# jixinya/EAMM

Hardware: AMD Instinct MI355X
Metric: 256x256 frames/sec (dense-motion + generator forward) (higher is better)
Workload: dtype f32; 1 GPU; 256x256, 10 keypoints, batch=16 synthetic frames per GPU per step, source encoded once per clip (BASELINE.json configs[2]); parallelism=frame-sharded x1

## Files before the change

eamm_amd/csrc/api_common.h:

```cpp
#pragma once
#include "../../include/eamm_hip.h"
#include "kernels.h"

#include <algorithm>
#include <cmath>
#include <cstdarg>
#include <cstdio>
#include <cstdlib>
#include <cstring>
#include <map>
#include <string>
#include <vector>

namespace eamm {

inline thread_local std::string g_create_error;

namespace {

struct HostTensor {
    std::vector<int64_t> shape;
    std::vector<float> data;
    size_t numel() const {
        size_t n = 1;
// ... 13 lines not shown


struct CtxBase {
    int device = 0;
    std::string err;
    std::map<std::string, HostTensor> sd;
    bool finalized = false;
    std::vector<void*> owned;
    int dma_min_m = 4608;
    int big_min_m = 49152;
    int dma_cfg_n256 = 2, dma_cfg_n128 = 2, dma_cfg_n64 = 3;
    int patch_poly = 1;
    int skinny_max_m = 16384;
    int patch_split_max = 4;
    int patch_min_blocks = 128;
};

struct DeviceGuard {
    int prev = -1;
    bool switched = false;
    hipError_t status = hipSuccess;
    explicit DeviceGuard(int device) {
        if (hipGetDevice(&prev) != hipSuccess) prev = -1;
        if (prev != device) {
            status = hipSetDevice(device);
            switched = status == hipSuccess && prev >= 0;
        }
    }
    ~DeviceGuard() {
        if (switched) (void)hipSetDevice(prev);
// ... 285 lines not shown
    if (int rc = fold_conv(c, {{conv, norm}}, 3, Cin_real, &f)) return rc;
    HostConv p = f;
    p.Cin = Cin_packed;
    p.w.assign((size_t)f.Cout * Cin_packed * 9, 0.f);
    for (int o = 0; o < f.Cout; ++o)
        std::copy_n(f.w.begin() + (size_t)o * Cin_real * 9, (size_t)Cin_real * 9, p.w.begin() + (size_t)o * Cin_packed * 9);
    return pack_wino(c, p, 4, L, false);
}

const ConvLayer& pick(const CtxBase* c, const LayerSet& S, size_t M) {
    if (S.has_skinny && M <= (size_t)c->skinny_max_m) return M <= 32 ? S.skinny32 : S.skinny64;
    if (S.has_big && M >= (size_t)c->big_min_m) return S.big;
    return (S.has_dma && M >= (size_t)c->dma_min_m) ? S.dma : S.base;
}

int launch_up(CtxBase* c, const LayerSet& S, const ConvIO& io, hipStream_t s) {
    if (S.has_patch) {
        int cus = 256;
        (void)hipDeviceGetAttribute(&cus, hipDeviceAttributeMultiprocessorCount, c->device);
        int splits = 1;
        if (S.patch.w_poly) {
            splits = patch_poly_splits(S.patch, io.B, io.Hin, io.Win, c->patch_split_max, cus);
            if ((size_t)splits * io.B * 4 * io.Hin * io.Win * S.patch.Cout > io.partial_cap) splits = 1;
        }
        const int blocks = ((io.Hin + 15) / 16) * ((io.Win + 15) / 16) * io.B * ((S.patch.Cout + 31) / 32) * splits;
        if (blocks >= c->patch_min_blocks && io.Hin >= 16 && io.Win >= 16 && io.act == ACT_RELU && !io.resid && !io.out2 && !io.pool && !io.nchw) {
            if (S.patch.w_poly)
                HIP_TRY(c, patch_poly_launch(S.patch, io.in0, io.in1, io.B, io.Hin, io.Win, io.act, io.out, s, splits, io.partial,
                                             io.partial_cap));
            else
                HIP_TRY(c, patch_phase_launch(S.patch, io.in0, io.in1, io.B, io.Hin, io.Win, io.act, io.out, s));
            return EAMM_OK;
        }
    }
    HIP_TRY(c, conv_launch(pick(c, S, (size_t)io.B * io.Hin * io.Win), io, s));
    return EAMM_OK;
}

int env_int(const char* name, int dflt) { return (int)knob_int(name, dflt); }

int round_up(int v, int m) { return (v + m - 1) / m * m; }

bool is_pow2(int v) { return v > 0 && (v & (v - 1)) == 0; }


inline void read_tile_knobs(CtxBase* c) {
    c->dma_min_m = env_int("EAMM_DMA_MIN_M", c->dma_min_m);
    c->big_min_m = env_int("EAMM_BIG_MIN_M", c->big_min_m);
    c->patch_poly = env_int("EAMM_PATCH_POLY", c->patch_poly);
    c->dma_cfg_n256 = env_int("EAMM_DMA_CFG_N256", c->dma_cfg_n256);
    c->dma_cfg_n128 = env_int("EAMM_DMA_CFG_N128", c->dma_cfg_n128);
    c->dma_cfg_n64 = env_int("EAMM_DMA_CFG_N64", c->dma_cfg_n64);
    c->patch_min_blocks = env_int("EAMM_PATCH_MIN_BLOCKS", c->patch_min_blocks);
    c->patch_split_max = env_int("EAMM_PATCH_SPLIT_MAX", c->patch_split_max);
    c->skinny_max_m = env_int("EAMM_SKINNY_MAX_M", c->skinny_max_m);
}

inline void free_owned(CtxBase* c) {
    DeviceGuard guard(c->device);
    (void)hipDeviceSynchronize();
    for (void* p : c->owned) (void)hipFree(p);
    c->owned.clear();
}

inline int store_tensor(CtxBase* c, const char* key, const float* host, const int64_t* shape, int ndim) {
    if (!c || !key || !host || ndim < 0 || (ndim > 0 && !shape)) return fail(c, EAMM_ERR_ARG, "null argument");
    if (c->finalized) return fail(c, EAMM_ERR_STATE, "weights already finalised; create a new handle to reload");
    HostTensor t;
    t.shape.assign(shape, shape + ndim);
// ... 29 lines not shown
```

eamm_amd/csrc/conv_mfma_patch_poly.hip:

```cpp
#include "conv_common.h"

#include <algorithm>
#include <cstdlib>
#include <cstring>

namespace eamm {

typedef __attribute__((address_space(3))) void* lds_ptr_t;

__device__ __forceinline__ f32x4 pk_sub4(f32x4 a, f32x4 b) {
    typedef float f32x2 __attribute__((ext_vector_type(2)));
    f32x2 alo = {a[0], a[1]}, ahi = {a[2], a[3]}, blo = {b[0], b[1]}, bhi = {b[2], b[3]}, rlo, rhi;
    asm("v_pk_add_f32 %0, %1, %2 neg_lo:[0,1] neg_hi:[0,1]" : "=v"(rlo) : "v"(alo), "v"(blo));
    asm("v_pk_add_f32 %0, %1, %2 neg_lo:[0,1] neg_hi:[0,1]" : "=v"(rhi) : "v"(ahi), "v"(bhi));
    return f32x4{rlo[0], rlo[1], rhi[0], rhi[1]};
}

namespace {
constexpr int ZT = 16;
constexpr int ZW = ZT + 2;
constexpr int ZPIX = ZW * ZW;
constexpr int ZPAD = (ZPIX + 7) / 8 * 8;
constexpr int ZBN = 32;
constexpr int ZWAVES = 8;
// ... 1 lines not shown

struct PatchPolyArgs {
    const float* in0;
    const float* in1;
    int C0, C1;
    unsigned in0_bytes, in1_bytes, w_bytes;
    int B, H, W;
    int tiles_x, tiles_y, ntiles;
    const float* w;
    const float* bias;
    int Cout, act;
    float* out;
    int splits;
    float* partial;
    size_t slab;
};

template <int FORM>
__global__ __launch_bounds__(ZWAVES * 64) void conv_patch_poly_kernel(const PatchPolyArgs p) {
    constexpr int BK = CONV_BK;
    constexpr int A_STAGE = ZPAD * BK;
    constexpr int B_STAGE = 9 * ZBN * BK;
    constexpr int A_PIECES = ZPAD / 8, B_PIECES = 9 * ZBN / 8;
    constexpr int A_INSTR = (A_PIECES + ZWAVES - 1) / ZWAVES;
    constexpr int B_INSTR = (B_PIECES + ZWAVES - 1) / ZWAVES;
    static_assert(A_INSTR + B_INSTR <= 12, "one DMA piece per sub-step");
    constexpr int B3_STAGE = 9 * 3 * 256;
    constexpr int B3_PIECES = 9 * 3, B3_INSTR = (B3_PIECES + ZWAVES - 1) / ZWAVES, A_HALF = A_INSTR / 2;
    static_assert(A_INSTR % 2 == 0 && B3_INSTR + A_HALF <= 9, "one DMA piece per point of a half-chunk");
    extern __shared__ __attribute__((aligned(16))) float smem[];
    float* const As = smem;
    float* const Bs = smem + 2 * A_STAGE;

    const int tid = threadIdx.x;
    const int lane = tid & 63;
    const int wave = __builtin_amdgcn_readfirstlane(tid >> 6);
    const int l31 = lane & 31, half = lane >> 5;

    int L = xcd_remap(blockIdx.x, gridDim.x);
    const int ntile = L % p.ntiles;
    L /= p.ntiles;
    const int ks = L % p.splits;
    L /= p.splits;
    const int tx0 = (L % p.tiles_x) * ZT;
    L /= p.tiles_x;
    const int ty0 = (L % p.tiles_y) * ZT;
    const int b = L / p.tiles_y;
    const int cchunks = (p.C0 + p.C1) / BK;
    const int c_begin = ks * cchunks / p.splits, c_end = (ks + 1) * cchunks / p.splits;

    const __amdgpu_buffer_rsrc_t rs0 = __builtin_amdgcn_make_buffer_rsrc((void*)p.in0, 0, p.in0_bytes, 0x00020000);
    const __amdgpu_buffer_rsrc_t rs1 =
        __builtin_amdgcn_make_buffer_rsrc((void*)(p.in1 ? p.in1 : p.in0), 0, p.in1 ? p.in1_bytes : 0u, 0x00020000);
    const __amdgpu_buffer_rsrc_t rsw = __builtin_amdgcn_make_buffer_rsrc((void*)p.w, 0, p.w_bytes, 0x00020000);
    constexpr unsigned OOB = 0xFFFFFFF0u;
    int pix[A_INSTR];
    static_for<A_INSTR>([&](auto jc) {
        constexpr int j = decltype(jc)::value;
        const int i = (wave + ZWAVES * j) * 8 + (lane >> 3);
        const int pyy = i / ZW, pxx = i - pyy * ZW;
        const int y = ty0 + pyy - 1, x = tx0 + pxx - 1;
        const bool ok = i < ZPIX && (unsigned)y < (unsigned)p.H && (unsigned)x < (unsigned)p.W;
        pix[j] = ok ? (b * p.H + y) * p.W + x : -1;
    });
    const unsigned slot_b = (unsigned)(((lane & 7) ^ ((((wave & 1) << 2) + (lane >> 4)) & 7)) << 4);
    auto dma_patch_piece = [&](auto jc, int cc, int st) {
        constexpr int j = decltype(jc)::value;
        if (wave + ZWAVES * j < A_PIECES) {
            const int c0 = cc * BK;
            const bool first = c0 < p.C0;
            const int C = first ? p.C0 : p.C1;
            const unsigned so = (unsigned)(first ? c0 : c0 - p.C0) * 4u;
            const int pj = pix[j];
            const unsigned vo = pj >= 0 ? (unsigned)(pj * C) * 4u + slot_b : OOB;
            float* dst = As + st * A_STAGE + (wave + ZWAVES * j) * (8 * BK);
            __builtin_amdgcn_raw_ptr_buffer_load_lds(first ? rs0 : rs1, (lds_ptr_t)dst, 16, vo, so, 0, 0);
        }
    };
    const unsigned w_lane = (unsigned)lane * 16u;
    auto dma_weight_piece = [&](auto jc, int cc, int st) {
        constexpr int j = decltype(jc)::value;
        if (wave + ZWAVES * j < B_PIECES) {
            const unsigned so = (unsigned)((ntile * cchunks + cc) * B_STAGE + (wave + ZWAVES * j) * (8 * BK)) * 4u;
            float* dst = Bs + st * B_STAGE + (wave + ZWAVES * j) * (8 * BK);
            __builtin_amdgcn_raw_ptr_buffer_load_lds(rsw, (lds_ptr_t)dst, 16, w_lane, so, 0, 0);
        }
    };

    auto dma_plane_piece = [&](auto jc, int hc, int wst) {
        constexpr int j = decltype(jc)::value;
        if (wave + ZWAVES * j < B3_PIECES) {
            const unsigned so = (unsigned)((ntile * 2 * cchunks + hc) * B3_STAGE + (wave + ZWAVES * j) * 256) * 4u;
            float* dst = Bs + wst * B3_STAGE + (wave + ZWAVES * j) * 256;
            __builtin_amdgcn_raw_ptr_buffer_load_lds(rsw, (lds_ptr_t)dst, 16, w_lane, so, 0, 0);
        }
    };

    f32x16 acc[9];
    static_for<9>([&](auto kc) {
        static_for<16>([&](auto rc) { acc[decltype(kc)::value][decltype(rc)::value] = 0.f; });
    });

    const int trow = 2 * wave + (l31 >> 4), tcol = ((l31 & 15) - 2 * (l31 >> 4)) & 15;
    const int idx0 = (trow + 1) * ZW + tcol + 1;
    int ta[9];
    static_for<9>([&](auto kc) {
        constexpr int k = decltype(kc)::value;
        const int idx = idx0 + (k / 3 - 1) * ZW + (k % 3 - 1);
        ta[k] = idx * BK + ((half ^ ((idx >> 1) & 7)) << 2);
    });
    const int bw0 = l31 * BK + ((half ^ ((l31 >> 1) & 7)) << 2);

    f32x4 x1[3];
    f32x4 xr[3];
    f32x4 v[2][3];
    f32x4 bb[2][3];
// ... 18 lines not shown
        v[q & 1][0] = r1;
        v[q & 1][1] = r0 - r1;
        v[q & 1][2] = r2 - r1;
    };
    auto mfmas = [&](auto qc, auto hc) {
        constexpr int q = decltype(qc)::value, i = q % 3, h = decltype(hc)::value;
        static_for<2>([&](auto tc) {
            constexpr int t = 2 * h + decltype(tc)::value;
            static_for<3>([&](auto jc) {
                constexpr int j = decltype(jc)::value;
                acc[3 * i + j] = __builtin_amdgcn_mfma_f32_32x32x2f32(v[q & 1][j][t], bb[q & 1][j][t], acc[3 * i + j], 0, 0, 0);
            });
        });
    };

    auto chunk = [&](int cc) {
        const int st = (cc - c_begin) & 1;
        const float* a_stage = As + st * A_STAGE;
        const float* b_stage = Bs + st * B_STAGE;
        const bool more = cc + 1 < c_end;
        fetch(std::integral_constant<int, 0>{}, a_stage, b_stage);
        transform(std::integral_constant<int, 0>{});
        static_for<12>([&](auto qc) {
            constexpr int q = decltype(qc)::value;
            if constexpr (q + 1 < 12) fetch(std::integral_constant<int, q + 1>{}, a_stage, b_stage);
            __builtin_amdgcn_sched_barrier(0);
            mfmas(qc, std::integral_constant<int, 0>{});
            __builtin_amdgcn_sched_barrier(0);
            if constexpr (q + 1 < 12) transform(std::integral_constant<int, q + 1>{});
            __builtin_amdgcn_sched_barrier(0);
            mfmas(qc, std::integral_constant<int, 1>{});
            if constexpr (q < B_INSTR) {
                if (more) dma_weight_piece(std::integral_constant<int, q>{}, cc + 1, st ^ 1);
            } else if constexpr (q - B_INSTR < A_INSTR) {
                if (more) dma_patch_piece(std::integral_constant<int, q - B_INSTR>{}, cc + 1, st ^ 1);
            }
            __builtin_amdgcn_sched_barrier(0);
        });
        asm volatile("s_waitcnt vmcnt(0)" ::: "memory");
        __syncthreads();
    };

    auto half_chunk = [&](int cc, auto Sc) {
        constexpr int S = decltype(Sc)::value;
        const int st = (cc - c_begin) & 1;
        const float* a_stage = As + st * A_STAGE;
        const float* b_stage = Bs + S * B3_STAGE + lane * 4;
        const bool more = cc + 1 < c_end;
        f32x4 xr[2], cr[2], r1[2];
        u32x4 ap[3], ub[3];
        auto load_raw = [&](auto ptc) {
            constexpr int pt = decltype(ptc)::value, i = pt / 3, j = pt % 3;
            constexpr int col = j == 0 ? 1 : j == 1 ? 0 : 2, row = i == 0 ? 1 : i == 1 ? 0 : 2;
            static_for<2>([&](auto hc) {
                constexpr int h2 = decltype(hc)::value;
                xr[h2] = *reinterpret_cast<const f32x4*>(a_stage + (ta[3 * row + col] ^ (8 * (2 * S + h2))));
                if constexpr (i > 0) cr[h2] = *reinterpret_cast<const f32x4*>(a_stage + (ta[3 + col] ^ (8 * (2 * S + h2))));
            });
        };
        auto load_planes = [&](auto ptc) {
            constexpr int pt = decltype(ptc)::value;
            static_for<3>([&](auto plc) {
                constexpr int pl = decltype(plc)::value;
// ... 14 lines not shown
        static_for<9>([&](auto ptc) {
            constexpr int pt = decltype(ptc)::value;
            load_planes(ptc);
            __builtin_amdgcn_sched_barrier(0);
            split_point(ptc);
            __builtin_amdgcn_sched_barrier(0);
            if constexpr (pt + 1 < 9) load_raw(std::integral_constant<int, pt + 1>{});
            __builtin_amdgcn_sched_barrier(0);
            static_for<SPLIT_TERMS>([&](auto tc) {
                constexpr int t = decltype(tc)::value;
                constexpr int pa = SPLIT_TERM_A[t], pb = SPLIT_TERM_B[t];
                acc[pt] = __builtin_amdgcn_mfma_f32_32x32x16_bf16(__builtin_bit_cast(bf16x8_t, ap[pa]),
                                                                  __builtin_bit_cast(bf16x8_t, ub[pb]), acc[pt], 0, 0, 0);
            });
            if constexpr (pt < B3_INSTR) {
                if (S == 0 || more) dma_plane_piece(std::integral_constant<int, pt>{}, 2 * cc + S + 1, S ^ 1);
            } else if constexpr (pt - B3_INSTR < A_HALF) {
                if (more) dma_patch_piece(std::integral_constant<int, A_HALF * S + pt - B3_INSTR>{}, cc + 1, st ^ 1);
            }
            __builtin_amdgcn_sched_barrier(0);
        });
        asm volatile("s_waitcnt vmcnt(0)" ::: "memory");
        __syncthreads();
    };

    static_for<A_INSTR>([&](auto jc) { dma_patch_piece(jc, c_begin, 0); });
    if constexpr (FORM == 1) static_for<B3_INSTR>([&](auto jc) { dma_plane_piece(jc, 2 * c_begin, 0); });
    else static_for<B_INSTR>([&](auto jc) { dma_weight_piece(jc, c_begin, 0); });
    asm volatile("s_waitcnt vmcnt(0)" ::: "memory");
    __syncthreads();
    if constexpr (FORM == 1) {
        for (int cc = c_begin; cc < c_end; ++cc) {
            half_chunk(cc, std::integral_constant<int, 0>{});
            half_chunk(cc, std::integral_constant<int, 1>{});
        }
    } else {
        for (int cc = c_begin; cc < c_end; ++cc) chunk(cc);
    }

    constexpr int LDO = ZBN + 4, C4 = ZBN / 4, NTHR = ZWAVES * 64, PER = ZT * ZT * C4 / NTHR;
    const int OH = 2 * p.H, OW = 2 * p.W;
    const bool raw = p.splits > 1;
    const float bias = raw ? 0.f : p.bias[ntile * ZBN + l31];
    float* const dst = raw ? p.partial + (size_t)ks * p.slab : p.out;
    static_for<4>([&](auto phc) {
        constexpr int ph = decltype(phc)::value, py = ph >> 1, px = ph & 1;
        if constexpr (ph > 0) __syncthreads();
        static_for<16>([&](auto rc) {
            constexpr int r = decltype(rc)::value;
            const int m = (r & 3) + 8 * (r >> 2) + 4 * half;
            const int pixel = (2 * wave + (m >> 4)) * ZT + (((m & 15) - 2 * (m >> 4)) & 15);
            const float y = (acc[0][r] + acc[1 + px][r]) + (acc[3 * (1 + py)][r] + acc[3 * (1 + py) + 1 + px][r]);
            smem[pixel * LDO + l31] = y + bias;
        });
        __syncthreads();
#pragma unroll
        for (int k = 0; k < PER; ++k) {
            const int idx = tid + k * NTHR;
            const int row = idx / C4, c4 = idx - row * C4;
            const int y = ty0 + (row >> 4), x = tx0 + (row & 15);
            const int n = ntile * ZBN + c4 * 4;
            if (y < p.H && x < p.W && n < p.Cout) {
                float4 o4 = *reinterpret_cast<const float4*>(smem + row * LDO + c4 * 4);
                if (!raw) {
                    o4.x = apply_act(o4.x, p.act); o4.y = apply_act(o4.y, p.act);
                    o4.z = apply_act(o4.z, p.act); o4.w = apply_act(o4.w, p.act);
                }
                const size_t o = ((size_t)(b * OH + 2 * y + py) * OW + 2 * x + px) * p.Cout + n;
                *reinterpret_cast<float4*>(dst + o) = o4;
            }
        }
    });
}

__global__ __launch_bounds__(256) void patch_poly_reduce_kernel(const float* __restrict__ partial, int splits, size_t slab,
                                                                const float* __restrict__ bias, int Cout, int act,
                                                                float* __restrict__ out, size_t total4) {
    const int c4n = Cout >> 2;
    for (size_t i = (size_t)blockIdx.x * blockDim.x + threadIdx.x; i < total4; i += (size_t)gridDim.x * blockDim.x) {
        float4 v = reinterpret_cast<const float4*>(partial)[i];
        for (int sp = 1; sp < splits; ++sp) {
            const float4 t = reinterpret_cast<const float4*>(partial + (size_t)sp * slab)[i];
            v.x += t.x; v.y += t.y; v.z += t.z; v.w += t.w;
        }
        const float4 bs = reinterpret_cast<const float4*>(bias)[i % c4n];
        v.x = apply_act(v.x + bs.x, act); v.y = apply_act(v.y + bs.y, act);
        v.z = apply_act(v.z + bs.z, act); v.w = apply_act(v.w + bs.w, act);
// ... 54 lines not shown
    const size_t total = 3 * patch_poly_packed_elems(cin_packed, Cout);
    for (size_t i = 0; i < total; ++i) dst[i] = 0;
    patch_poly_for_each_u(w, Cout, Cin, cin_map, cin_packed, [&](int o, int cp, int pt, float u) {
        const int nt = o / ZBN, nl = o % ZBN;
        const int hc = cp / 16, kl = cp % 16;
        const int lane = ((kl >> 2) & 1) * 32 + nl, e = (kl >> 3) * 4 + (kl & 3);
        uint16_t pl[3];
        split3_bf16_host(u, pl);
        uint16_t* blk = dst + ((((size_t)nt * hch + hc) * 9 + pt) * 3) * 512 + lane * 8 + e;
        for (int k = 0; k < 3; ++k) blk[k * 512] = pl[k];
    });
}

size_t patch_poly_split_packed_elems(int Cin_packed, int Cout) { return patch_poly_packed_elems(Cin_packed, Cout) * 3 / 2; }

hipError_t patch_poly_launch(const PatchLayer& L, const float* in0, const float* in1, int B, int H, int W, int act,
                              float* out, hipStream_t stream, int splits, float* partial, size_t partial_cap) {
    if ((L.C0 % CONV_BK) || (L.C1 % CONV_BK) || (L.Cout & 3) || L.w_poly == nullptr) return hipErrorInvalidValue;
    const size_t slab = (size_t)B * 4 * H * W * L.Cout;
    if (splits < 1 || (splits > 1 && (partial == nullptr || (size_t)splits * slab > partial_cap))) return hipErrorInvalidValue;
    PatchPolyArgs a{};
    a.in0 = in0;
    a.in1 = L.C1 ? in1 : nullptr;
    a.C0 = L.C0;
    a.C1 = L.C1;
    const size_t px = (size_t)B * H * W;
    const bool split = splits == 1 && L.w_poly3 != nullptr;
    const size_t b0 = px * L.C0 * 4, b1 = px * L.C1 * 4,
                 bw = (split ? patch_poly_split_packed_elems(L.C0 + L.C1, L.Cout) : patch_poly_packed_elems(L.C0 + L.C1, L.Cout)) * 4;
    if (b0 >= 0xFFFFFFF0ull || b1 >= 0xFFFFFFF0ull || bw >= 0xFFFFFFF0ull) return hipErrorInvalidValue;
    a.in0_bytes = (unsigned)b0;
    a.in1_bytes = (unsigned)b1;
    a.w_bytes = (unsigned)bw;
    a.B = B;
    a.H = H;
    a.W = W;
    a.tiles_x = (W + ZT - 1) / ZT;
    a.tiles_y = (H + ZT - 1) / ZT;
    a.ntiles = (L.Cout + ZBN - 1) / ZBN;
    a.w = split ? L.w_poly3 : L.w_poly;
    a.bias = L.bias;
    a.Cout = L.Cout;
    a.act = act;
    a.out = out;
    a.splits = splits;
    a.partial = partial;
    a.slab = slab;
    constexpr size_t lds_loop0 = sizeof(float) * 2 * (ZPAD * CONV_BK + 9 * ZBN * CONV_BK);
    constexpr size_t lds_loop1 = sizeof(float) * 2 * (ZPAD * CONV_BK + 9 * 3 * 256);
    constexpr size_t lds_epi = sizeof(float) * (ZT * ZT) * (ZBN + 4);
    static_assert(lds_loop0 <= 160 * 1024 && lds_loop0 >= lds_loop1 && lds_loop1 >= lds_epi, "LDS budget");
    const size_t lds = split ? lds_loop1 : lds_loop0;
    static lds_once_mask configured[2] = {{0}, {0}};
    const auto kern = split ? conv_patch_poly_kernel<1> : conv_patch_poly_kernel<0>;
    if (hipError_t e = ensure_dynamic_lds(kern, lds, &configured[split]); e != hipSuccess) return e;
    const int blocks = a.tiles_x * a.tiles_y * B * a.ntiles * splits;
    note_mfma_flops(2.0 * a.tiles_x * a.tiles_y * B * (ZT * ZT) * 9.0 * (a.ntiles * ZBN) * (L.C0 + L.C1));
    hipLaunchKernelGGL(kern, dim3(blocks), dim3(ZWAVES * 64), lds, stream, a);
    if (splits > 1) {
        const size_t total4 = slab / 4;
        const int rb = (int)std::min<size_t>((total4 + 255) / 256, 4096);
        hipLaunchKernelGGL(patch_poly_reduce_kernel, dim3(rb), dim3(256), 0, stream, partial, splits, slab, L.bias, L.Cout, act, out,
                           total4);
    }
    return hipGetLastError();
}

}
```

eamm_amd/csrc/eamm_forward.hip:

```cpp
#include "eamm_ctx.h"
#include <mutex>

namespace {
constexpr int POOL_MAXDEV = 64, POOL_MAXCHAIN = 15;
std::mutex g_pool_mu;
hipStream_t g_pool[POOL_MAXDEV][POOL_MAXCHAIN] = {};
std::mutex g_pool_lease[POOL_MAXDEV];

}

hipStream_t chain_stream(int device, int k) {
    if (device < 0 || device >= POOL_MAXDEV || k < 0 || k >= POOL_MAXCHAIN) return nullptr;
    std::lock_guard<std::mutex> lock(g_pool_mu);
    if (!g_pool[device][k] && hipStreamCreateWithFlags(&g_pool[device][k], hipStreamNonBlocking) != hipSuccess) g_pool[device][k] = nullptr;
    return g_pool[device][k];
}

FrameView make_view(const eamm_ctx* c, int f0, int n, int ns_call, int slab, const float* kd_val, const float* kd_jac,
                    const float* ks_val, const float* ks_jac, const eamm_outputs* o) {
    FrameView v;
    const size_t F = (size_t)f0, K = c->K;
    const size_t HW = (size_t)c->H * c->W, hw = (size_t)c->h * c->w, hwf = (size_t)c->hf * c->wf;
    const size_t sf = ns_call > 1 ? F : 0;
    v.n = n;
// ... 412 lines not shown
    const eamm_outputs* const user = o;
    eamm_outputs staged = *o;
    if (o->frames_u8 && c->Cimg != 3) return fail(c, EAMM_ERR_ARG, "uint8 RGB frames need num_channels == 3");
    if (c->Cimg < 3) {
        if (o->frames_u8) return fail(c, EAMM_ERR_ARG, "uint8 RGB frames need num_channels == 3");
        staged.prediction = c->stage_pred;
        if (o->deformed) staged.deformed = c->stage_deformed;
        if (o->sparse_deformed) staged.sparse_deformed = c->stage_sparse;
        o = &staged;
    }

    StreamLease lease(c, s);
    if (lease.rc) return lease.rc;
    const int chains = pass_chains(c, n);
    c->cur_call_frames = n;
    c->prof.begin_call(n, chains);
    if (chains == 1) {
        if (int rc = forward_view(c, make_view(c, 0, n, ns, 0, kd_val, kd_jac, ks_val, ks_jac, o), s, 0, false)) return rc;
    } else {
        const int nbase = n / chains, nrem = n % chains;
        HIP_TRY(c, hipEventRecord(c->ev_fork, s));
        for (int k = 1; k < chains; ++k) HIP_TRY(c, hipStreamWaitEvent(c->side_streams[k - 1], c->ev_fork, 0));
        for (int k = 0; k < chains; ++k) {
            const int nk = nbase + (k < nrem ? 1 : 0), f0 = k * nbase + std::min(k, nrem);
            const FrameView v = make_view(c, f0, nk, ns, k, kd_val, kd_jac, ks_val, ks_jac, o);
            if (int rc = forward_view(c, v, k ? c->side_streams[k - 1] : s, k, true)) return rc;
        }
        for (int k = 1; k < chains; ++k) {
            HIP_TRY(c, hipEventRecord(c->ev_join[k - 1], c->side_streams[k - 1]));
            HIP_TRY(c, hipStreamWaitEvent(s, c->ev_join[k - 1], 0));
// ... 146 lines not shown
```

eamm_amd/csrc/eamm_op_conv.hip:

```cpp
#include "op_common.h"

namespace {

struct ConvOp {
    const float *in0, *in1;
    int C0, C1, B, Hin, Win, up;
    const float *w, *b;
    int Cout, kh, kw, act, pool;
    const float* resid;
    int splitk, tile_n;
    float* out;
    int iters;
    float* avg_ms;
    const float *pre_s, *pre_t;
    float* out2;
    const float *s2, *t2;
    int nchw, split_n;
    const char* name;
    hipStream_t s;
};

const char* conv_refusal(const ConvOp& a) {
    const bool staged = a.tile_n == 0 || a.tile_n == 32 || a.tile_n == 64 || a.tile_n == 128;
    const bool gemm = staged || (a.tile_n > 1000 && a.tile_n <= 1005);
// ... 52 lines not shown
    if (a.kh != 7 || a.kw != 1 || a.up || a.pool || a.resid || a.splitk > 1 || a.Cout != bn || a.act != 0 || a.C0 % 32 || a.C1 % 32 ||
        (!streamed && (a.C1 || a.C0 > 64)))
        return fail(t, EAMM_ERR_ARG, "%s: unsupported column-patch configuration", a.name);
    float* w = nullptr;
    if (int rc = upload_conv_image(t, &w, op_weights(a, a.C0 + a.C1, false), nullptr, a.C0 + a.C1, bn, MODE_PLAIN, true)) return rc;
    auto col7 = [&]() {
        return streamed ? conv_col7s_launch(a.in0, a.C0, a.in1, a.C1, a.B, a.Hin, a.Win, w, 3, a.out, 96, a.s)
                        : conv_col7_launch(a.in0, a.C0, a.B, a.Hin, a.Win, w, a.out, a.s);
    };
    HIP_TRY(t, col7());
    HIP_TRY(t, time_launches(a.s, a.iters, a.avg_ms, col7));
    return EAMM_OK;
}

int op_conv_patch(OpBuffers* t, const ConvOp& a) {
    const bool pp = a.tile_n == 3003 || a.tile_n == 3004;
    const int psplit = a.splitk > 1 ? a.splitk : 1;
    if (a.kh != 3 || a.kw != 3 || !a.up || a.pool || a.resid || (a.Cout & 3) || (psplit > 1 && (!pp || ((a.C0 + a.C1) / 32) % psplit)))
        return fail(t, EAMM_ERR_ARG, "%s: unsupported patch-kernel configuration", a.name);
    PatchLayer P;
    float* ppart = nullptr;
    const size_t ppart_elems = psplit > 1 ? (size_t)psplit * a.B * 4 * a.Hin * a.Win * a.Cout : 0;
    int rc = pack_patch(t, op_weights(a, a.C0 + a.C1), nullptr, a.C0, a.C1, pp, &P, a.tile_n == 3003);
    if (rc || (psplit > 1 && (rc = dev_alloc(t, &ppart, ppart_elems)))) return rc;
    auto patch = [&]() {
        return pp ? patch_poly_launch(P, a.in0, a.in1, a.B, a.Hin, a.Win, a.act, a.out, a.s, psplit, ppart, ppart_elems)
                  : patch_phase_launch(P, a.in0, a.in1, a.B, a.Hin, a.Win, a.act, a.out, a.s);
    };
    HIP_TRY(t, patch());
    HIP_TRY(t, time_launches(a.s, a.iters, a.avg_ms, patch));
    return EAMM_OK;
}

int op_conv_wino(OpBuffers* t, const ConvOp& a) {
    const bool w4 = a.tile_n >= 2100;
    const int w4_groups = a.tile_n >= 2150 ? a.tile_n - 2150 : 1;
    const int w4_variant = w4_groups > 1 ? 0 : a.tile_n - 2100;
    if ((!w4 && a.tile_n != 2000) || a.kh != 3 || a.kw != 3 || a.up || (a.pool && (w4_groups == 1 || a.resid)) || a.C1 || a.splitk > 1 || a.C0 % 64 ||
        (a.Cout & 3) || (w4 && ((a.Hin & 3) || (a.Win & 3))))
        return fail(t, EAMM_ERR_ARG, "%s: unsupported Winograd configuration", a.name);
    WinoLayer W;
    float *V = nullptr, *Zb = nullptr;
    int rc = pack_wino(t, op_weights(a, a.C0), w4 ? 4 : 2, &W);
    if (rc || (rc = dev_alloc(t, &V, (size_t)16 * a.B * (a.Hin / 2) * (a.Win / 2) * a.C0))) return rc;
// ... 37 lines not shown
    io.out2 = a.out2;
    io.s2 = a.s2;
    io.t2 = a.t2;
    io.split_n = a.split_n;
    if (io.partial_cap && (rc = dev_alloc(t, &io.partial, io.partial_cap))) return rc;
    auto gemm = [&]() { return conv_launch(L, io, a.s, a.splitk); };
    HIP_TRY(t, gemm());
    HIP_TRY(t, time_launches(a.s, a.iters, a.avg_ms, gemm));
    return EAMM_OK;
}

int op_conv_run(OpBuffers* t, const ConvOp& a) {
    int rc;
    if (a.tile_n == 4002 || a.tile_n == 4003) rc = op_conv_final(t, a);
    else if (a.tile_n == 4000 || a.tile_n == 4001) rc = op_conv_col7(t, a);
    else if (a.tile_n == 3000 || a.tile_n == 3003 || a.tile_n == 3004) rc = op_conv_patch(t, a);
    else if (a.tile_n >= 2000 && a.tile_n < 2200) rc = op_conv_wino(t, a);
    else rc = op_conv_gemm(t, a);
    if (rc) return rc;
    HIP_TRY(t, hipStreamSynchronize(a.s));
    return EAMM_OK;
}

int op_conv_call(int device, ConvOp a, void* stream_) {
    if (const char* why = conv_refusal(a)) return fail(nullptr, EAMM_ERR_ARG, "%s: %s", a.name, why);
    DeviceGuard guard(device);
    if (guard.status != hipSuccess) return fail(nullptr, EAMM_ERR_HIP, "hipSetDevice failed");
    a.s = reinterpret_cast<hipStream_t>(stream_);
    OpBuffers t(device, a.s);
    if (int rc = op_conv_run(&t, a)) return fail(nullptr, rc, "%s", t.err.c_str());
    return EAMM_OK;
// ... 84 lines not shown
```

eamm_amd/csrc/kernels.h:

```cpp
#pragma once
#include <hip/hip_runtime.h>
#include <stddef.h>
#include <stdint.h>

namespace eamm {

constexpr int CONV_BK = 32;
constexpr int CONV_LDK = CONV_BK + 4;
inline size_t round64(size_t n) { return (n + 63) / 64 * 64; }
constexpr int KP_STRIDE = 8;

enum Act { ACT_NONE = 0, ACT_RELU = 1, ACT_SIGMOID = 2 };

void note_mfma_flops(double flops);
double take_mfma_flops();
double total_mfma_flops();

long long knob_int(const char* name, long long dflt);
int knobs_json(char* buf, int cap);

struct ConvArgs {
    const float* in0;
    const float* in1;
    int C0, C1;
// ... 59 lines not shown
hipError_t conv_launch(const ConvLayer& L, const ConvIO& io, hipStream_t stream, int force_splits = 0);

struct PatchLayer {
    int C0 = 0, C1 = 0, Cout = 0;
    float* w = nullptr;
    float* w_poly = nullptr;
    float* w_poly3 = nullptr;
    float* bias = nullptr;
};
size_t patch_packed_elems(int Cin_packed, int Cout);
size_t patch_poly_packed_elems(int Cin_packed, int Cout);
void patch_poly_pack_host(const float* w_oihw_3x3, int Cout, int Cin, const int* cin_map, int cin_packed, float* dst);
size_t patch_poly_split_packed_elems(int Cin_packed, int Cout);
void patch_poly_pack_split_host(const float* w_oihw_3x3, int Cout, int Cin, const int* cin_map, int cin_packed, uint16_t* dst);
hipError_t patch_poly_launch(const PatchLayer& L, const float* in0, const float* in1, int B, int H, int W, int act,
                             float* out, hipStream_t stream, int splits = 1, float* partial = nullptr, size_t partial_cap = 0);
int patch_poly_splits(const PatchLayer& L, int B, int H, int W, int max_splits, int cus);
void patch_pack_host(const float* w_oihw_3x3, int Cout, int Cin, const int* cin_map, int cin_packed, float* dst);
hipError_t patch_phase_launch(const PatchLayer& L, const float* in0, const float* in1, int B, int H, int W, int act,
                              float* out, hipStream_t stream);

hipError_t conv_col7_launch(const float* in, int C, int B, int H, int W, const float* w_swizzled, float* out,
                            hipStream_t stream);
hipError_t conv_col7_fused_launch(const float* in, int C, int B, int H, int W, const float* w_swizzled, const float* bias,
                                  float* out_nchw, hipStream_t stream, const float* w_split = nullptr);
size_t col7_split_packed_elems(int cin_packed);
void col7_pack_split_host(const float* w_rowsplit, int Cout, int Cin, const int* cin_map, int cin_packed, uint16_t* dst);

hipError_t final_shift_sum_launch(const float* part , const float* bias ,
                                  int n, int H, int W, float* out , hipStream_t s);
hipError_t conv_col7s_launch(const float* in0, int C0, const float* in1, int C1, int B, int H, int W, const float* w_swizzled,
// ... 279 lines not shown
```

Measured before the change: 4419 frames/s.

## Make patch-poly upsample conv persistent, walking unit ranges with cross-unit prefetch

The patch-poly upsampling conv kernel becomes persistent. Each workgroup now walks a contiguous range of (ntile, split, tile, batch) units, and the grid is capped at the CU count, or that count divided by the concurrent chains. While the last channel chunk of one unit computes, the kernel prefetches the first weight and patch chunk of the next unit, so the per-block prologue DMA stall and launch overhead are hidden across units. The trade-offs are extra index bookkeeping, less parallelism when there are few units, and possible load imbalance. Optional cycle-stamp instrumentation is added behind an experiments flag.

```diff
diff --git a/eamm_amd/csrc/api_common.h b/eamm_amd/csrc/api_common.h
--- a/eamm_amd/csrc/api_common.h
+++ b/eamm_amd/csrc/api_common.h
@@ -51,6 +51,8 @@
     int skinny_max_m = 16384;
     int patch_split_max = 4;
     int patch_min_blocks = 128;
+    int patch_walk = 1;
+    int concurrent_chains = 1;
 };
 
 struct DeviceGuard {
@@ -366,6 +368,11 @@
     return (S.has_dma && M >= (size_t)c->dma_min_m) ? S.dma : S.base;
 }
 
+inline int patch_walk_wgs(int mode, int cus, int chains, int splits) {
+    if (mode <= 0 || splits > 1) return 0;
+    return mode == 1 ? cus : std::max(1, cus / std::max(1, chains));
+}
+
 int launch_up(CtxBase* c, const LayerSet& S, const ConvIO& io, hipStream_t s) {
     if (S.has_patch) {
         int cus = 256;
@@ -379,7 +386,7 @@
         if (blocks >= c->patch_min_blocks && io.Hin >= 16 && io.Win >= 16 && io.act == ACT_RELU && !io.resid && !io.out2 && !io.pool && !io.nchw) {
             if (S.patch.w_poly)
                 HIP_TRY(c, patch_poly_launch(S.patch, io.in0, io.in1, io.B, io.Hin, io.Win, io.act, io.out, s, splits, io.partial,
-                                             io.partial_cap));
+                                             io.partial_cap, patch_walk_wgs(c->patch_walk, cus, c->concurrent_chains, splits)));
             else
                 HIP_TRY(c, patch_phase_launch(S.patch, io.in0, io.in1, io.B, io.Hin, io.Win, io.act, io.out, s));
             return EAMM_OK;
@@ -405,6 +412,7 @@
     c->dma_cfg_n64 = env_int("EAMM_DMA_CFG_N64", c->dma_cfg_n64);
     c->patch_min_blocks = env_int("EAMM_PATCH_MIN_BLOCKS", c->patch_min_blocks);
     c->patch_split_max = env_int("EAMM_PATCH_SPLIT_MAX", c->patch_split_max);
+    c->patch_walk = env_int("EAMM_PATCH_WALK", c->patch_walk);
     c->skinny_max_m = env_int("EAMM_SKINNY_MAX_M", c->skinny_max_m);
 }
 
diff --git a/eamm_amd/csrc/conv_mfma_patch_poly.hip b/eamm_amd/csrc/conv_mfma_patch_poly.hip
--- a/eamm_amd/csrc/conv_mfma_patch_poly.hip
+++ b/eamm_amd/csrc/conv_mfma_patch_poly.hip
@@ -39,10 +39,25 @@
     int splits;
     float* partial;
     size_t slab;
+    int units;
+    int units_q, units_r;
+    long long* stamps;
 };
 
-template <int FORM>
+struct PatchPolyUnit {
+    int nk;
+    int tyx;
+    int b;
+    __device__ int ntile() const { return nk & 0xFFFF; }
+    __device__ int ks() const { return nk >> 16; }
+    __device__ int tx0() const { return tyx & 0xFFFF; }
+    __device__ int ty0() const { return tyx >> 16; }
+};
+
+template <int FORM_>
 __global__ __launch_bounds__(ZWAVES * 64) void conv_patch_poly_kernel(const PatchPolyArgs p) {
+    constexpr int FORM = FORM_ & 1;
+    constexpr bool STAMP = FORM_ >= 2;
     constexpr int BK = CONV_BK;
     constexpr int A_STAGE = ZPAD * BK;
     constexpr int B_STAGE = 9 * ZBN * BK;
@@ -62,17 +77,44 @@
     const int wave = __builtin_amdgcn_readfirstlane(tid >> 6);
     const int l31 = lane & 31, half = lane >> 5;
 
-    int L = xcd_remap(blockIdx.x, gridDim.x);
-    const int ntile = L % p.ntiles;
-    L /= p.ntiles;
-    const int ks = L % p.splits;
-    L /= p.splits;
-    const int tx0 = (L % p.tiles_x) * ZT;
-    L /= p.tiles_x;
-    const int ty0 = (L % p.tiles_y) * ZT;
-    const int b = L / p.tiles_y;
+    auto per_unit_args = [&]() {
+        auto* q = (const __attribute__((address_space(4))) PatchPolyArgs*)__builtin_amdgcn_kernarg_segment_ptr();
+        asm volatile("" : "+s"(q));
+        return q;
+    };
+
+    const int L = xcd_remap(blockIdx.x, gridDim.x);
+    auto range_begin = [&](int l) { return l * p.units_q + (p.units_r ? (int)((unsigned)(l * p.units_r) / gridDim.x) : 0); };
+    const int u0 = range_begin(L);
+    int left = range_begin(L + 1) - u0;
+    if (left <= 0) return;
+    PatchPolyUnit cur;
+    {
+        int t = u0;
+        cur.nk = t % p.ntiles;
+        t /= p.ntiles;
+        cur.nk |= (t % p.splits) << 16;
+        t /= p.splits;
+        cur.tyx = (t % p.tiles_x) * ZT;
+        t /= p.tiles_x;
+        cur.tyx |= (t % p.tiles_y) * ZT << 16;
+        cur.b = t / p.tiles_y;
+    }
+    auto successor = [&](PatchPolyUnit n) {
+        const auto* q = per_unit_args();
+        if ((++n.nk & 0xFFFF) < q->ntiles) return n;
+        n.nk = (n.nk & ~0xFFFF) + 0x10000;
+        if (n.ks() < q->splits) return n;
+        n.nk = 0;
+        if ((n.tyx += ZT, n.tx0()) < q->tiles_x * ZT) return n;
+        n.tyx = (n.tyx & ~0xFFFF) + (ZT << 16);
+        if (n.ty0() < q->tiles_y * ZT) return n;
+        n.tyx = 0;
+        ++n.b;
+        return n;
+    };
     const int cchunks = (p.C0 + p.C1) / BK;
-    const int c_begin = ks * cchunks / p.splits, c_end = (ks + 1) * cchunks / p.splits;
+    auto chunk_begin = [&](const PatchPolyUnit& n) { return n.ks() * (cchunks / per_unit_args()->splits); };
 
     const __amdgpu_buffer_rsrc_t rs0 = __builtin_amdgcn_make_buffer_rsrc((void*)p.in0, 0, p.in0_bytes, 0x00020000);
     const __amdgpu_buffer_rsrc_t rs1 =
@@ -80,14 +122,21 @@
     const __amdgpu_buffer_rsrc_t rsw = __builtin_amdgcn_make_buffer_rsrc((void*)p.w, 0, p.w_bytes, 0x00020000);
     constexpr unsigned OOB = 0xFFFFFFF0u;
     int pix[A_INSTR];
-    static_for<A_INSTR>([&](auto jc) {
-        constexpr int j = decltype(jc)::value;
-        const int i = (wave + ZWAVES * j) * 8 + (lane >> 3);
-        const int pyy = i / ZW, pxx = i - pyy * ZW;
-        const int y = ty0 + pyy - 1, x = tx0 + pxx - 1;
-        const bool ok = i < ZPIX && (unsigned)y < (unsigned)p.H && (unsigned)x < (unsigned)p.W;
-        pix[j] = ok ? (b * p.H + y) * p.W + x : -1;
-    });
+    auto patch_pixels = [&](const PatchPolyUnit& n) {
+        const auto* q = per_unit_args();
+        const int H = q->H, W = q->W;
+        int le = lane;
+        asm volatile("" : "+v"(le));
+        static_for<A_INSTR>([&](auto jc) {
+            constexpr int j = decltype(jc)::value;
+            const int i = (wave + ZWAVES * j) * 8 + (le >> 3);
+            const int pyy = i / ZW, pxx = i - pyy * ZW;
+            const int y = n.ty0() + pyy - 1, x = n.tx0() + pxx - 1;
+            const bool ok = i < ZPIX && (unsigned)y < (unsigned)H && (unsigned)x < (unsigned)W;
+            pix[j] = ok ? (n.b * H + y) * W + x : -1;
+        });
+    };
+    patch_pixels(cur);
     const unsigned slot_b = (unsigned)(((lane & 7) ^ ((((wave & 1) << 2) + (lane >> 4)) & 7)) << 4);
     auto dma_patch_piece = [&](auto jc, int cc, int st) {
         constexpr int j = decltype(jc)::value;
@@ -103,7 +152,7 @@
         }
     };
     const unsigned w_lane = (unsigned)lane * 16u;
-    auto dma_weight_piece = [&](auto jc, int cc, int st) {
+    auto dma_weight_piece = [&](auto jc, int ntile, int cc, int st) {
         constexpr int j = decltype(jc)::value;
         if (wave + ZWAVES * j < B_PIECES) {
             const unsigned so = (unsigned)((ntile * cchunks + cc) * B_STAGE + (wave + ZWAVES * j) * (8 * BK)) * 4u;
@@ -112,7 +161,7 @@
         }
     };
 
-    auto dma_plane_piece = [&](auto jc, int hc, int wst) {
+    auto dma_plane_piece = [&](auto jc, int ntile, int hc, int wst) {
         constexpr int j = decltype(jc)::value;
         if (wave + ZWAVES * j < B3_PIECES) {
             const unsigned so = (unsigned)((ntile * 2 * cchunks + hc) * B3_STAGE + (wave + ZWAVES * j) * 256) * 4u;
@@ -122,9 +171,6 @@
     };
 
     f32x16 acc[9];
-    static_for<9>([&](auto kc) {
-        static_for<16>([&](auto rc) { acc[decltype(kc)::value][decltype(rc)::value] = 0.f; });
-    });
 
     const int trow = 2 * wave + (l31 >> 4), tcol = ((l31 & 15) - 2 * (l31 >> 4)) & 15;
     const int idx0 = (trow + 1) * ZW + tcol + 1;
@@ -173,11 +219,9 @@
         });
     };
 
-    auto chunk = [&](int cc) {
-        const int st = (cc - c_begin) & 1;
+    auto chunk = [&](int cc, int st, bool more, int nnt, int ncc) {
         const float* a_stage = As + st * A_STAGE;
         const float* b_stage = Bs + st * B_STAGE;
-        const bool more = cc + 1 < c_end;
         fetch(std::integral_constant<int, 0>{}, a_stage, b_stage);
         transform(std::integral_constant<int, 0>{});
         static_for<12>([&](auto qc) {
@@ -190,9 +234,9 @@
             __builtin_amdgcn_sched_barrier(0);
             mfmas(qc, std::integral_constant<int, 1>{});
             if constexpr (q < B_INSTR) {
-                if (more) dma_weight_piece(std::integral_constant<int, q>{}, cc + 1, st ^ 1);
+                if (more) dma_weight_piece(std::integral_constant<int, q>{}, nnt, ncc, st ^ 1);
             } else if constexpr (q - B_INSTR < A_INSTR) {
-                if (more) dma_patch_piece(std::integral_constant<int, q - B_INSTR>{}, cc + 1, st ^ 1);
+                if (more) dma_patch_piece(std::integral_constant<int, q - B_INSTR>{}, ncc, st ^ 1);
             }
             __builtin_amdgcn_sched_barrier(0);
         });
@@ -200,12 +244,10 @@
         __syncthreads();
     };
 
-    auto half_chunk = [&](int cc, auto Sc) {
+    auto half_chunk = [&](int cc, auto Sc, int st, bool more, int nnt, int ncc) {
         constexpr int S = decltype(Sc)::value;
-        const int st = (cc - c_begin) & 1;
         const float* a_stage = As + st * A_STAGE;
         const float* b_stage = Bs + S * B3_STAGE + lane * 4;
-        const bool more = cc + 1 < c_end;
         f32x4 xr[2], cr[2], r1[2];
         u32x4 ap[3], ub[3];
         auto load_raw = [&](auto ptc) {
@@ -250,9 +292,10 @@
                                                                   __builtin_bit_cast(bf16x8_t, ub[pb]), acc[pt], 0, 0, 0);
             });
             if constexpr (pt < B3_INSTR) {
-                if (S == 0 || more) dma_plane_piece(std::integral_constant<int, pt>{}, 2 * cc + S + 1, S ^ 1);
+                if constexpr (S == 0) dma_plane_piece(std::integral_constant<int, pt>{}, cur.ntile(), 2 * cc + 1, 1);
+                else if (more) dma_plane_piece(std::integral_constant<int, pt>{}, nnt, 2 * ncc, 0);
             } else if constexpr (pt - B3_INSTR < A_HALF) {
-                if (more) dma_patch_piece(std::integral_constant<int, A_HALF * S + pt - B3_INSTR>{}, cc + 1, st ^ 1);
+                if (more) dma_patch_piece(std::integral_constant<int, A_HALF * S + pt - B3_INSTR>{}, ncc, st ^ 1);
             }
             __builtin_amdgcn_sched_barrier(0);
         });
@@ -260,53 +303,95 @@
         __syncthreads();
     };
 
+    constexpr int LDO = ZBN + 4, C4 = ZBN / 4, NTHR = ZWAVES * 64, PER = ZT * ZT * C4 / NTHR;
+    static_assert(ZT * ZT * LDO <= A_STAGE, "the epilogue stages in one patch stage");
+    constexpr int STAMP_WGS = 8, STAMP_UNITS = 8;
+    long long ts0 = 0, ts1 = 0, ts2 = 0;
+    if constexpr (STAMP) ts0 = __builtin_readcyclecounter();
+    const int c_begin = chunk_begin(cur);
     static_for<A_INSTR>([&](auto jc) { dma_patch_piece(jc, c_begin, 0); });
-    if constexpr (FORM == 1) static_for<B3_INSTR>([&](auto jc) { dma_plane_piece(jc, 2 * c_begin, 0); });
-    else static_for<B_INSTR>([&](auto jc) { dma_weight_piece(jc, c_begin, 0); });
+    if constexpr (FORM == 1) static_for<B3_INSTR>([&](auto jc) { dma_plane_piece(jc, cur.ntile(), 2 * c_begin, 0); });
+    else static_for<B_INSTR>([&](auto jc) { dma_weight_piece(jc, cur.ntile(), c_begin, 0); });
     asm volatile("s_waitcnt vmcnt(0)" ::: "memory");
     __syncthreads();
-    if constexpr (FORM == 1) {
-        for (int cc = c_begin; cc < c_end; ++cc) {
-            half_chunk(cc, std::integral_constant<int, 0>{});
-            half_chunk(cc, std::integral_constant<int, 1>{});
-        }
-    } else {
-        for (int cc = c_begin; cc < c_end; ++cc) chunk(cc);
+    int st = 0;
+    for (int ui = 0;; ++ui) {
+        if constexpr (STAMP) ts1 = __builtin_readcyclecounter();
+        const bool has_next = left > 1;
+        const PatchPolyUnit nxt = has_next ? successor(cur) : cur;
+        const int c_first = chunk_begin(cur), c_end = c_first + cchunks / per_unit_args()->splits;
+        static_for<9>([&](auto kc) {
+            static_for<16>([&](auto rc) { acc[decltype(kc)::value][decltype(rc)::value] = 0.f; });
+        });
+        for (int cc = c_first; cc < c_end; ++cc, st ^= 1) {
+            const bool last = cc + 1 == c_end;
+            if (last && has_next) patch_pixels(nxt);
+            const bool more = !last || has_next;
+            int nnt = cur.ntile(), ncc = cc + 1;
+            if (last && has_next) {
+                nnt = nxt.ntile();
+                ncc = chunk_begin(nxt);
+            }
+            if constexpr (FORM == 1) {
+                half_chunk(cc, std::integral_constant<int, 0>{}, st, more, nnt, ncc);
+                half_chunk(cc, std::integral_constant<int, 1>{}, st, more, nnt, ncc);
+            } else {
+                chunk(cc, st, more, nnt, ncc);
+            }
+        }
+        if constexpr (STAMP) ts2 = __builtin_readcyclecounter();
+
+        float* const stage = As + (st ^ 1) * A_STAGE;
+        int l31e = l31, halfe = half, tide = tid;
+        asm volatile("" : "+v"(l31e), "+v"(halfe), "+v"(tide));
+        const auto* q = per_unit_args();
+        const int ntile = cur.ntile(), ty0 = cur.ty0(), tx0 = cur.tx0(), b = cur.b;
+        const int H = q->H, W = q->W, OH = 2 * H, OW = 2 * W, Cout = q->Cout, act = q->act;
+        const bool raw = q->splits > 1;
+        const float bias = raw ? 0.f : q->bias[ntile * ZBN + l31e];
+        float* const dst = raw ? q->partial + (size_t)cur.ks() * q->slab : q->out;
+        static_for<4>([&](auto phc) {
+            constexpr int ph = decltype(phc)::value, py = ph >> 1, px = ph & 1;
+            if constexpr (ph > 0) __syncthreads();
+            static_for<16>([&](auto rc) {
+                constexpr int r = decltype(rc)::value;
+                const int m = (r & 3) + 8 * (r >> 2) + 4 * halfe;
+                const int pixel = (2 * wave + (m >> 4)) * ZT + (((m & 15) - 2 * (m >> 4)) & 15);
+                const float y = (acc[0][r] + acc[1 + px][r]) + (acc[3 * (1 + py)][r] + acc[3 * (1 + py) + 1 + px][r]);
+                stage[pixel * LDO + l31e] = y + bias;
+            });
+            __syncthreads();
+#pragma unroll
+            for (int k = 0; k < PER; ++k) {
+                const int idx = tide + k * NTHR;
+                const int row = idx / C4, c4 = idx - row * C4;
+                const int y = ty0 + (row >> 4), x = tx0 + (row & 15);
+                const int n = ntile * ZBN + c4 * 4;
+                if (y < H && x < W && n < Cout) {
+                    float4 o4 = *reinterpret_cast<const float4*>(stage + row * LDO + c4 * 4);
+                    if (!raw) {
+                        o4.x = apply_act(o4.x, act); o4.y = apply_act(o4.y, act);
+                        o4.z = apply_act(o4.z, act); o4.w = apply_act(o4.w, act);
+                    }
+                    const size_t o = ((size_t)(b * OH + 2 * y + py) * OW + 2 * x + px) * Cout + n;
+                    *reinterpret_cast<float4*>(dst + o) = o4;
+                }
+            }
+        });
+        if constexpr (STAMP) {
+            asm volatile("s_waitcnt vmcnt(0)" ::: "memory");
+            const long long ts3 = __builtin_readcyclecounter();
+            if (p.stamps != nullptr && tid == 0 && L < STAMP_WGS && ui < STAMP_UNITS) {
+                long long* o = p.stamps + (L * STAMP_UNITS + ui) * 4;
+                o[0] = ts0; o[1] = ts1; o[2] = ts2; o[3] = ts3;
+            }
+        }
+        if (!has_next) break;
+        __syncthreads();
+        if constexpr (STAMP) ts0 = __builtin_readcyclecounter();
+        cur = nxt;
+        --left;
     }
-
-    constexpr int LDO = ZBN + 4, C4 = ZBN / 4, NTHR = ZWAVES * 64, PER = ZT * ZT * C4 / NTHR;
-    const int OH = 2 * p.H, OW = 2 * p.W;
-    const bool raw = p.splits > 1;
-    const float bias = raw ? 0.f : p.bias[ntile * ZBN + l31];
-    float* const dst = raw ? p.partial + (size_t)ks * p.slab : p.out;
-    static_for<4>([&](auto phc) {
-        constexpr int ph = decltype(phc)::value, py = ph >> 1, px = ph & 1;
-        if constexpr (ph > 0) __syncthreads();
-        static_for<16>([&](auto rc) {
-            constexpr int r = decltype(rc)::value;
-            const int m = (r & 3) + 8 * (r >> 2) + 4 * half;
-            const int pixel = (2 * wave + (m >> 4)) * ZT + (((m & 15) - 2 * (m >> 4)) & 15);
-            const float y = (acc[0][r] + acc[1 + px][r]) + (acc[3 * (1 + py)][r] + acc[3 * (1 + py) + 1 + px][r]);
-            smem[pixel * LDO + l31] = y + bias;
-        });
-        __syncthreads();
-#pragma unroll
-        for (int k = 0; k < PER; ++k) {
-            const int idx = tid + k * NTHR;
-            const int row = idx / C4, c4 = idx - row * C4;
-            const int y = ty0 + (row >> 4), x = tx0 + (row & 15);
-            const int n = ntile * ZBN + c4 * 4;
-            if (y < p.H && x < p.W && n < p.Cout) {
-                float4 o4 = *reinterpret_cast<const float4*>(smem + row * LDO + c4 * 4);
-                if (!raw) {
-                    o4.x = apply_act(o4.x, p.act); o4.y = apply_act(o4.y, p.act);
-                    o4.z = apply_act(o4.z, p.act); o4.w = apply_act(o4.w, p.act);
-                }
-                const size_t o = ((size_t)(b * OH + 2 * y + py) * OW + 2 * x + px) * p.Cout + n;
-                *reinterpret_cast<float4*>(dst + o) = o4;
-            }
-        }
-    });
 }
 
 __global__ __launch_bounds__(256) void patch_poly_reduce_kernel(const float* __restrict__ partial, int splits, size_t slab,
@@ -391,8 +476,21 @@
 
 size_t patch_poly_split_packed_elems(int Cin_packed, int Cout) { return patch_poly_packed_elems(Cin_packed, Cout) * 3 / 2; }
 
+#ifdef EAMM_EXPERIMENTS
+namespace {
+long long* g_stamps = nullptr;
+}
+void patch_poly_set_stamps(long long* dev) { g_stamps = dev; }
+int patch_poly_stamp_slots(int* wgs, int* units) {
+    *wgs = 8;
+    *units = 8;
+    return 4;
+}
+#endif
+
 hipError_t patch_poly_launch(const PatchLayer& L, const float* in0, const float* in1, int B, int H, int W, int act,
-                              float* out, hipStream_t stream, int splits, float* partial, size_t partial_cap) {
+                              float* out, hipStream_t stream, int splits, float* partial, size_t partial_cap, int walk_wgs) {
+    if (walk_wgs < 0 || H >= 32768 || W >= 32768 || L.Cout > 0xFFFF * ZBN) return hipErrorInvalidValue;
     if ((L.C0 % CONV_BK) || (L.C1 % CONV_BK) || (L.Cout & 3) || L.w_poly == nullptr) return hipErrorInvalidValue;
     const size_t slab = (size_t)B * 4 * H * W * L.Cout;
     if (splits < 1 || (splits > 1 && (partial == nullptr || (size_t)splits * slab > partial_cap))) return hipErrorInvalidValue;
@@ -423,15 +521,28 @@
     a.splits = splits;
     a.partial = partial;
     a.slab = slab;
+    a.units = a.tiles_x * a.tiles_y * B * a.ntiles * splits;
+    if ((L.C0 + L.C1) / CONV_BK % splits) return hipErrorInvalidValue;
+    a.stamps = nullptr;
     constexpr size_t lds_loop0 = sizeof(float) * 2 * (ZPAD * CONV_BK + 9 * ZBN * CONV_BK);
     constexpr size_t lds_loop1 = sizeof(float) * 2 * (ZPAD * CONV_BK + 9 * 3 * 256);
     constexpr size_t lds_epi = sizeof(float) * (ZT * ZT) * (ZBN + 4);
     static_assert(lds_loop0 <= 160 * 1024 && lds_loop0 >= lds_loop1 && lds_loop1 >= lds_epi, "LDS budget");
     const size_t lds = split ? lds_loop1 : lds_loop0;
-    static lds_once_mask configured[2] = {{0}, {0}};
-    const auto kern = split ? conv_patch_poly_kernel<1> : conv_patch_poly_kernel<0>;
-    if (hipError_t e = ensure_dynamic_lds(kern, lds, &configured[split]); e != hipSuccess) return e;
-    const int blocks = a.tiles_x * a.tiles_y * B * a.ntiles * splits;
+    static lds_once_mask configured[4] = {{0}, {0}, {0}, {0}};
+    auto kern = split ? conv_patch_poly_kernel<1> : conv_patch_poly_kernel<0>;
+    int which = split;
+#ifdef EAMM_EXPERIMENTS
+    if (g_stamps != nullptr) {
+        a.stamps = g_stamps;
+        kern = split ? conv_patch_poly_kernel<3> : conv_patch_poly_kernel<2>;
+        which += 2;
+    }
+#endif
+    if (hipError_t e = ensure_dynamic_lds(kern, lds, &configured[which]); e != hipSuccess) return e;
+    const int blocks = walk_wgs > 0 ? std::min(a.units, std::min(walk_wgs, 65535)) : a.units;
+    a.units_q = a.units / blocks;
+    a.units_r = a.units % blocks;
     note_mfma_flops(2.0 * a.tiles_x * a.tiles_y * B * (ZT * ZT) * 9.0 * (a.ntiles * ZBN) * (L.C0 + L.C1));
     hipLaunchKernelGGL(kern, dim3(blocks), dim3(ZWAVES * 64), lds, stream, a);
     if (splits > 1) {
diff --git a/eamm_amd/csrc/eamm_forward.hip b/eamm_amd/csrc/eamm_forward.hip
--- a/eamm_amd/csrc/eamm_forward.hip
+++ b/eamm_amd/csrc/eamm_forward.hip
@@ -450,6 +450,7 @@
     if (lease.rc) return lease.rc;
     const int chains = pass_chains(c, n);
     c->cur_call_frames = n;
+    c->concurrent_chains = chains;
     c->prof.begin_call(n, chains);
     if (chains == 1) {
         if (int rc = forward_view(c, make_view(c, 0, n, ns, 0, kd_val, kd_jac, ks_val, ks_jac, o), s, 0, false)) return rc;
diff --git a/eamm_amd/csrc/eamm_op_conv.hip b/eamm_amd/csrc/eamm_op_conv.hip
--- a/eamm_amd/csrc/eamm_op_conv.hip
+++ b/eamm_amd/csrc/eamm_op_conv.hip
@@ -90,20 +90,49 @@
 }
 
 int op_conv_patch(OpBuffers* t, const ConvOp& a) {
-    const bool pp = a.tile_n == 3003 || a.tile_n == 3004;
+    const bool pp = a.tile_n >= 3003 && a.tile_n <= 3006;
     const int psplit = a.splitk > 1 ? a.splitk : 1;
     if (a.kh != 3 || a.kw != 3 || !a.up || a.pool || a.resid || (a.Cout & 3) || (psplit > 1 && (!pp || ((a.C0 + a.C1) / 32) % psplit)))
         return fail(t, EAMM_ERR_ARG, "%s: unsupported patch-kernel configuration", a.name);
     PatchLayer P;
     float* ppart = nullptr;
     const size_t ppart_elems = psplit > 1 ? (size_t)psplit * a.B * 4 * a.Hin * a.Win * a.Cout : 0;
-    int rc = pack_patch(t, op_weights(a, a.C0 + a.C1), nullptr, a.C0, a.C1, pp, &P, a.tile_n == 3003);
+    int rc = pack_patch(t, op_weights(a, a.C0 + a.C1), nullptr, a.C0, a.C1, pp, &P, pp && a.tile_n != 3004);
     if (rc || (psplit > 1 && (rc = dev_alloc(t, &ppart, ppart_elems)))) return rc;
+    int cus = 256;
+    (void)hipDeviceGetAttribute(&cus, hipDeviceAttributeMultiprocessorCount, t->device);
+    const int walk_env = env_int("EAMM_OP_PATCH_WALK_WGS", -1);
+    const int walk = a.tile_n == 3005 ? 0 : a.tile_n == 3006 ? 3 : walk_env >= 0 ? walk_env : patch_walk_wgs(t->patch_walk, cus, 1, psplit);
     auto patch = [&]() {
-        return pp ? patch_poly_launch(P, a.in0, a.in1, a.B, a.Hin, a.Win, a.act, a.out, a.s, psplit, ppart, ppart_elems)
+        return pp ? patch_poly_launch(P, a.in0, a.in1, a.B, a.Hin, a.Win, a.act, a.out, a.s, psplit, ppart, ppart_elems, walk)
                   : patch_phase_launch(P, a.in0, a.in1, a.B, a.Hin, a.Win, a.act, a.out, a.s);
     };
     HIP_TRY(t, patch());
+#ifdef EAMM_EXPERIMENTS
+    if (pp && env_int("EAMM_OP_PPOLY_STAMPS", 0) == 1) {
+        int wgs = 0, units = 0;
+        const int per = patch_poly_stamp_slots(&wgs, &units);
+        std::vector<long long> h((size_t)wgs * units * per, 0);
+        long long* d = nullptr;
+        HIP_TRY(t, hipMalloc((void**)&d, h.size() * sizeof(long long)));
+        HIP_TRY(t, hipMemsetAsync(d, 0, h.size() * sizeof(long long), a.s));
+        patch_poly_set_stamps(d);
+        const hipError_t e = patch();
+        patch_poly_set_stamps(nullptr);
+        if (e == hipSuccess) HIP_TRY(t, hipStreamSynchronize(a.s));
+        if (e == hipSuccess) HIP_TRY(t, hipMemcpy(h.data(), d, h.size() * sizeof(long long), hipMemcpyDeviceToHost));
+        (void)hipFree(d);
+        HIP_TRY(t, e);
+        for (int w = 0; w < wgs; ++w)
+            for (int u = 0; u < units; ++u) {
+                const long long* s4 = &h[((size_t)w * units + u) * per];
+                if (s4[3] == 0) continue;
+                printf("ppoly_stamps wg %d unit %d: prologue %lld loop %lld epilogue %lld cycles\n", w, u, s4[1] - s4[0], s4[2] - s4[1],
+                       s4[3] - s4[2]);
+            }
+        fflush(stdout);
+    }
+#endif
     HIP_TRY(t, time_launches(a.s, a.iters, a.avg_ms, patch));
     return EAMM_OK;
 }
@@ -171,7 +200,7 @@
     int rc;
     if (a.tile_n == 4002 || a.tile_n == 4003) rc = op_conv_final(t, a);
     else if (a.tile_n == 4000 || a.tile_n == 4001) rc = op_conv_col7(t, a);
-    else if (a.tile_n == 3000 || a.tile_n == 3003 || a.tile_n == 3004) rc = op_conv_patch(t, a);
+    else if (a.tile_n == 3000 || (a.tile_n >= 3003 && a.tile_n <= 3006)) rc = op_conv_patch(t, a);
     else if (a.tile_n >= 2000 && a.tile_n < 2200) rc = op_conv_wino(t, a);
     else rc = op_conv_gemm(t, a);
     if (rc) return rc;
diff --git a/eamm_amd/csrc/kernels.h b/eamm_amd/csrc/kernels.h
--- a/eamm_amd/csrc/kernels.h
+++ b/eamm_amd/csrc/kernels.h
@@ -97,7 +97,12 @@
 size_t patch_poly_split_packed_elems(int Cin_packed, int Cout);
 void patch_poly_pack_split_host(const float* w_oihw_3x3, int Cout, int Cin, const int* cin_map, int cin_packed, uint16_t* dst);
 hipError_t patch_poly_launch(const PatchLayer& L, const float* in0, const float* in1, int B, int H, int W, int act,
-                             float* out, hipStream_t stream, int splits = 1, float* partial = nullptr, size_t partial_cap = 0);
+                             float* out, hipStream_t stream, int splits = 1, float* partial = nullptr, size_t partial_cap = 0,
+                             int walk_wgs = 0);
+#ifdef EAMM_EXPERIMENTS
+void patch_poly_set_stamps(long long* dev);
+int patch_poly_stamp_slots(int* wgs, int* units);
+#endif
 int patch_poly_splits(const PatchLayer& L, int B, int H, int W, int max_splits, int cus);
 void patch_pack_host(const float* w_oihw_3x3, int Cout, int Cin, const int* cin_map, int cin_packed, float* dst);
 hipError_t patch_phase_launch(const PatchLayer& L, const float* in0, const float* in1, int B, int H, int W, int act,
```

Result: no change. 4433 frames/s, median of 5 (+0.3%).
